# cbs228/sameold

Hardware: AMD Instinct MI355X
Metric: Msamples/s demodulated (batched 22.05 kHz channels) + % HBM roofline, 1/8 GPU (higher is better)
Workload: dtype f32

## Files before the change

### sameold_amd/csrc/same_batch.cpp

```cpp
#include <hip/hip_runtime.h>

#include <algorithm>
#include <chrono>
#include <cstdarg>
#include <cstdio>
#include <cstdlib>
#include <condition_variable>
#include <cstring>
#include <deque>
#include <functional>
#include <mutex>
#include <new>
#include <string>
#include <thread>
#include <utility>
#include <vector>

#include "../../include/same_rx.h"
#include "same_config.h"
#include "same_device.h"
#include "same_hipmem.h"
#include "same_launch.h"
#include "same_resets.h"
#include "same_transport.h"
// ... 191 lines not shown
        uint64_t end_counter = 0;
        bool chunked = false;
        same::ChunkGeom geom{};
        uint64_t end_blocks = 0;
        same::DevBuf<uint64_t> d_handover;
        same::PinnedBuf<uint64_t> h_handover;
        bool per_channel = false;
        same::DevBuf<uint32_t> d_geom;
        same::PinnedBuf<uint32_t> h_geom;
        same::CoherentBuf<uint32_t> h_reset;
        same::CoherentBuf<uint32_t> h_counts;
        same::PinnedBuf<uint64_t> h_wake_up;
        bool dev_transport = false;
        same::CoherentBuf<same::DevMessage> h_near;
        uint32_t near_cap() const { return (uint32_t)h_near.size(); }
        same::DevBuf<same::DevMessage> d_msgs;
        uint32_t msg_cap() const { return (uint32_t)d_msgs.size(); }
        same::PinnedBuf<void> h_msgs;
        bool captured = false;
        same::DevBuf<same::cap::Span> d_spans;
        uint32_t span_cap() const { return (uint32_t)d_spans.size(); }
        same::DevBuf<float> d_pool;
        same::DevBuf<same::cap::Cursors> d_cap_cur;
        same::MappedBuf<same::cap::Cursors> h_cap_cur;
        same::PinnedBuf<void> h_spans, h_pool;
    } slot[2];
    struct TimePar {
        bool enabled = false;
        uint32_t max_chunks = 0, min_own = 0, warmup = 0;
        uint32_t cap_columns = 0;
        uint32_t carved_columns = 0;
        int carved_family = -1;
        same::Params Pv{};
        same::State Sv{};
        same::DevBuf<void> blob;
        same::DevBuf<void> blob_fresh;
        size_t fresh_bytes = 0;
        same::DevBuf<same::StateArrayDesc> d_desc_in, d_desc_out;
        uint32_t n_desc = 0;
        same::DevBuf<uint32_t> d_final_col;
        same::DevBuf<float> d_energy;
        same::DevBuf<float> d_hist;
        same::Event ev_plan_prev; bool plan_recorded = false;
        int knob_plan_stream = 0;
        int sort_mode = -1;
        uint32_t last_chunks = 1;
        bool last_per_channel = false;
        same::Family family = same::Family::kPipe;
        int knob_prologue = 0;
        std::vector<int64_t> sym_off;
        std::vector<TickSynth> synth;
    } tp;
    uint64_t launch_seq = 0;
    hipStream_t copy_stream = nullptr;
    struct Windowed {
        bool on = false;
        uint32_t window = 0;
        uint32_t fill = 0;
        same::DevBuf<void> d_buf;
        same::Event ev_buf;
        hipStream_t buf_stream = nullptr; bool buf_used = false;
        same::Event ev_read[2];
        uint64_t n_reads = 0;
        hipStream_t read_stream = nullptr;
    } inv;
    hipStream_t plan_stream = nullptr;
    float last_ms = 0.0f;
    bool overflowed = false;
    std::string record_path;
    bool kernel_fault = false;
    same::Request want;
    same::Mode mode;
    same::Choice plain;
    same::Params Pfm{};
    same::Family last_family = same::Family::kGeneric;
    bool sym_launched = false;
    bool debug = false;
    int host_threads = 0;
    same::DevBuf<void> d_stage, d_stage2;
    same::DevBuf<void> d_upload;
    same::DevBuf<void> d_zero;
    same::Event ev_order;
// ... 94 lines not shown
{
    out.clear();
#define DESC_ROWS(field, type, rows)                                                                     \
    out.push_back(same::StateArrayDesc{reinterpret_cast<char *>(src.field), reinterpret_cast<char *>(dst.field), \
                                       (uint32_t)(rows), (uint32_t)(sizeof(type) / 4)});
    SAME_STATE_ARRAYS(DESC_ROWS, P)
#undef DESC_ROWS
    static_assert(same::kBurstCap % 4 == 0, "framer rows are copied in words");
    out.push_back(same::StateArrayDesc{reinterpret_cast<char *>(src.fr_msg), reinterpret_cast<char *>(dst.fr_msg), 1u,
                                       (uint32_t)(same::kBurstCap / 4)});
}

void read_knobs(same_batch *rx)
{
    auto num = [](const char *name, int unset) { const char *e = std::getenv(name); return e ? std::atoi(e) : unset; };
    auto tri = [](const char *name) { const char *e = std::getenv(name); return e ? (std::atoi(e) ? 1 : -1) : 0; };
    rx->P.knob_pipe = tri("SAME_PIPE");
    rx->P.knob_pipe_lanes = num("SAME_PIPE_LANES", 0);
    rx->P.knob_pipe_split = tri("SAME_PIPE_SPLIT");
#ifdef SAME_PROFILE
    rx->P.knob_mirror = tri("SAME_MIRROR");
    rx->P.knob_pipe_share = tri("SAME_PIPE_SHARE");
    rx->P.knob_prio = num("SAME_PIPE_PRIO", 0);
#endif
    rx->P.knob_fast_dense = tri("SAME_FAST_DENSE");
    rx->P.knob_sym = tri("SAME_SYM");
    rx->want.sym_max_channels = (uint32_t)std::max(0, num("SAME_SYM_MAX", 1 << 30));
    rx->debug = std::getenv("SAME_DEBUG") != nullptr;
    { const char *e = std::getenv("SAME_RECORD_HARVEST"); rx->record_path = e ? e : ""; }
    rx->host_threads = std::max(0, num("SAME_HOST_THREADS", 0));
    rx->tp.sort_mode = num("SAME_TP_SORT", -1);
    rx->tp.knob_plan_stream = tri("SAME_TP_PLAN_STREAM");
    rx->tp.knob_prologue = tri("SAME_TP_PROLOGUE");
    rx->want.knob_relaxed = tri("SAME_RELAXED");
    { const char *e = std::getenv("SAME_RELAXED_KERNEL"); rx->P.knob_relaxed_kernel = !e ? 0 : (std::strcmp(e, "solo") == 0 ? 1 : (std::strcmp(e, "duo") == 0 ? 2 : 0)); }
    { const char *e = std::getenv("SAME_TP_KERNEL"); rx->want.knob_tp_kernel = !e ? 0 : (std::strcmp(e, "wave") == 0 ? 2 : (std::strcmp(e, "pipe") == 0 ? 1 : 0)); }
}

int ensure_output(same_batch *rx, same_batch::Slot &sl, size_t n_samples, same::Output &O, size_t n_columns = 0)
{
    const size_t n_ch = n_columns ? n_columns : rx->P.n_channels;
    const double symbols = (double)n_samples * 520.83 / (double)rx->P.input_rate;
    const size_t per_chan_events = (size_t)(symbols / 8.0) + 16;
    const size_t per_chan_bursts = (size_t)(symbols / 160.0) + 4;
    size_t ecap = std::min<size_t>(per_chan_events * n_ch, 0x7fffffffu / sizeof(same::DevEvent));
    size_t bcap = std::min<size_t>(per_chan_bursts * n_ch, 0x7fffffffu / same::kBurstCap);
    HIP_TRY(sl.d_events.ensure(ecap));
    HIP_TRY(sl.d_bursts.ensure(bcap * same::kBurstCap));
    if (rx->dev_transport && !n_columns) {
        HIP_TRY(sl.d_msgs.ensure(std::min<size_t>(bcap + 2 * n_ch, 0x7fffffffu / sizeof(same::DevMessage))));
        if (!sl.h_near) HIP_TRY(sl.h_near.ensure(std::max<uint32_t>(4096u, (uint32_t)(n_ch / 4u))));
        if (rx->audio.per_launch)
            HIP_TRY(sl.d_spans.ensure(std::min<size_t>(n_ch + (size_t)sl.near_cap() + sl.msg_cap(), 0x7fffffffu / sizeof(same::cap::Span))));
    }
    HIP_TRY(sl.d_sorted.ensure(sl.d_events.size()));
    HIP_TRY(sl.d_sort.ensure(2 * n_ch + 1 + same::event_sort_extra_words((uint32_t)n_ch)));
    HIP_TRY(sl.h_sort.ensure(n_ch + 1));
    sl.sort_bins = (uint32_t)n_ch;
    O.events = sl.d_events; O.event_cap = sl.event_cap();
    O.bursts = sl.d_bursts; O.burst_cap = sl.burst_cap();
    O.n_events = sl.d_counters; O.n_bursts = sl.d_counters + 1; O.overflow = sl.d_counters + 2;
    return SAME_OK;
}

template <typename SampleT>
hipError_t launch_family(same::Family f, const same::Params &P, const same::State &S, const same::Output &O, const float4 *taps, const SampleT *x,
// ... 618 lines not shown
        const uint64_t min_own = tp.min_own ? tp.min_own : 4ull * WB * fb;
        if (SB == 0 || SB * fb < min_own) return false;
        geom.counter0 = rx->counter;
        geom.n_chunks = K; geom.block_len = fb; geom.stride_blocks = (uint32_t)SB; geom.warmup_blocks = WB;
        pc.n_chunks = K; pc.in_channels = C; pc.stride_blocks = (uint32_t)SB; pc.nominal_blocks = (uint32_t)SB + WB;
        pc.handover = nullptr;
        return true;
    };
    const same::TpRule rule = same::tp_rule(rx->P, rx->mode, rx->want, tp.max_chunks, column_cap, channel_major);
    for (uint32_t K = rule.k_max; K >= 2u; --K) {
        same::Choice c;
        if (same::tp_candidate(rx->P, rule, K, c) && fill(K, c.block_len)) { tp.family = c.family; return K; }
    }
    return 1;
}

int ensure_handover(same_batch::Slot &sl, uint32_t columns)
{
    HIP_TRY(sl.d_handover.ensure(columns));
    HIP_TRY(sl.h_handover.ensure(columns));
    return SAME_OK;
}

int ensure_wide_state(same_batch *rx, uint32_t columns)
{
    same_batch::TimePar &tp = rx->tp;
    if (tp.carved_columns == columns && tp.carved_family == (int)tp.family) return SAME_OK;
    int rc = harvest(rx);
    if (rc) return rc;
    HIP_TRY(hipDeviceSynchronize());
    tp.Pv = same::wide_params(rx->P, columns, same::is_fastmath(tp.family), same::tp_more_than_one_round(columns));
    if (columns > tp.cap_columns) {
        tp.cap_columns = 0;
        HIP_TRY(tp.blob.reset());
        HIP_TRY(tp.blob_fresh.reset());
        const size_t bytes = carve_state(tp.Pv, nullptr, tp.Sv);
        HIP_TRY(tp.blob.ensure(bytes));
        HIP_TRY(hipMemset(tp.blob, 0, bytes));
        HIP_TRY(tp.blob_fresh.ensure(bytes));
        tp.cap_columns = columns;
    }
    const size_t blob_bytes = carve_state(tp.Pv, (char *)tp.blob.get(), tp.Sv);
    {
        same::State Sf{};
        carve_state(tp.Pv, (char *)tp.blob_fresh.get(), Sf);
        HIP_TRY(hipMemset(tp.blob_fresh, 0, blob_bytes));
        HIP_TRY(same::launch_init_state(tp.Pv, Sf, 0, nullptr, 0));
        HIP_TRY(hipDeviceSynchronize());
        tp.fresh_bytes = (size_t)(reinterpret_cast<char *>(tp.Sv.fr_msg) - static_cast<char *>(tp.blob.get()));
    }
    std::vector<same::StateArrayDesc> in, out;
    list_state_arrays(rx->P, rx->S, tp.Sv, in);
    list_state_arrays(rx->P, tp.Sv, rx->S, out);
    tp.n_desc = (uint32_t)in.size();
    HIP_TRY(tp.d_desc_in.ensure(in.size()));
    HIP_TRY(tp.d_desc_out.ensure(out.size()));
    HIP_TRY(tp.d_final_col.ensure(rx->P.n_channels));
    HIP_TRY(hipMemcpy(tp.d_desc_in, in.data(), in.size() * sizeof(same::StateArrayDesc), hipMemcpyHostToDevice));
    HIP_TRY(hipMemcpy(tp.d_desc_out, out.data(), out.size() * sizeof(same::StateArrayDesc), hipMemcpyHostToDevice));
    tp.carved_columns = columns;
    tp.carved_family = (int)tp.family;
    return SAME_OK;
}

struct Ragged {
    const uint32_t *counts = nullptr;
    uint32_t m = 0;
    uint32_t row_off = 0;
};

struct RaggedLaunch {
    uint32_t row0 = 0;
    size_t n_lock = 0;
};


int begin_launch(same_batch *rx, same_batch::Slot &sl, const same_batch::Slot &prev, hipStream_t stream)
{
    int rc = harvest_slot(rx, sl);
    if (rc) return rc;
    if (prev.in_flight && rx->last_stream != stream) HIP_TRY(hipStreamWaitEvent(stream, prev.ev_done, 0));
    return launch_pending_resets(rx, sl, stream);
}

int begin_timing(same_batch *rx, same_batch::Slot &sl, hipStream_t stream)
{
    sl.timed = rx->timing;
    if (sl.timed) HIP_TRY(hipEventRecord(sl.ev_start, stream));
    return SAME_OK;
}

int tp_reserve(same_batch *rx, same_batch::Slot &sl, uint32_t columns, size_t n, const same::PipeChunks &pc, uint32_t block_len, same::Output &O)
{
    int rc = ensure_wide_state(rx, columns);
    if (rc) return rc;
    rc = ensure_output(rx, sl, std::min<size_t>(n, 3 * (size_t)pc.nominal_blocks * block_len + 65536), O, columns);
    if (rc) return rc;
    return ensure_handover(sl, columns);
}

int tp_start(same_batch *rx, same_batch::Slot &sl, uint32_t columns, const char *layout, hipStream_t stream, bool *sort_bins_empty)
{
    same_batch::TimePar &tp = rx->tp;
    const uint32_t C = rx->P.n_channels;
    *sort_bins_empty = false;
    if (tp.knob_prologue >= 0) {
        HIP_TRY(same::launch_tp_prologue(tp.blob, tp.blob_fresh, tp.fresh_bytes, sl.d_handover, sl.d_sort, columns, sl.d_counters, stream));
        *sort_bins_empty = sl.sort_bins == columns;
    } else {
        HIP_TRY(same::launch_counters(sl.d_counters, sl.h_counters.dev(), 0, stream));
        HIP_TRY(same::launch_init_state(tp.Pv, tp.Sv, 0, stream, C));
        HIP_TRY(same::launch_fill_u64(sl.d_handover, columns, same::kNoHandover, stream));
    }
    if (rx->debug) std::fprintf(stderr, "[same] time-parallel launch: %u columns (%s), start-up: %s\n", columns, layout,
                                tp.knob_prologue >= 0 ? "prologue kernel" : "separate launches");
    HIP_TRY(same::launch_copy_state_columns(tp.d_desc_in, tp.n_desc, C, columns, nullptr, C, stream));
    return SAME_OK;
}

int tp_hand_back(same_batch *rx, same_batch::Slot &sl, const same::ChunkGeom &geom, const uint32_t *own_start, hipStream_t stream)
{
    same_batch::TimePar &tp = rx->tp;
    const uint32_t C = rx->P.n_channels;
    if (own_start) HIP_TRY(same::launch_chunk_final_column_pc(sl.d_handover, own_start, C, geom.n_chunks, rx->counter, tp.d_final_col, stream));
    else HIP_TRY(same::launch_chunk_final_column(sl.d_handover, C, geom, tp.d_final_col, stream));
    HIP_TRY(same::launch_copy_state_columns(tp.d_desc_out, tp.n_desc, geom.n_chunks * C, C, tp.d_final_col, C, stream));
    return SAME_OK;
}

template <typename SampleT>
int demod_tail(same_batch *rx, const same::Output &O, const SampleT *rows, size_t n, uint64_t counter0, hipStream_t stream)
{
    const hipError_t e = same::launch_demod(rx->P, rx->S, O, rx->d_taps, rows, (uint32_t)n, counter0, stream);
    if (e != hipSuccess) return fail(SAME_EHIP, "demod kernel launch failed: %s", hipGetErrorString(e));
    return SAME_OK;
}
int demod_tail_corner(same_batch *rx, const same::Output &O, const float *corner, size_t pitch, size_t r, uint64_t counter0, hipStream_t stream)
{
    const uint32_t C = rx->P.n_channels;
    HIP_TRY(rx->d_stage.ensure(r * C * sizeof(float)));
    HIP_TRY(rx->d_stage2.ensure(r * C * sizeof(float)));
    float *staged = static_cast<float *>(rx->d_stage.get()), *rows = static_cast<float *>(rx->d_stage2.get());
    HIP_TRY(hipMemcpy2DAsync(staged, r * sizeof(float), corner, pitch * sizeof(float), r * sizeof(float), C, hipMemcpyDeviceToDevice, stream));
    const hipError_t e = same::launch_transpose(staged, rows, C, (uint32_t)r, stream);
    if (e != hipSuccess) return fail(SAME_EHIP, "demod kernel launch failed: %s", hipGetErrorString(e));
    return demod_tail(rx, O, rows, r, counter0, stream);
}

template <typename SampleT>
int end_launch(same_batch *rx, same_batch::Slot &sl, same_batch::Slot &prev, hipStream_t stream, const SampleT *rows, size_t n,
               bool sort_bins_empty, const RaggedLaunch *rl = nullptr)
{
    if (sl.timed) HIP_TRY(hipEventRecord(sl.ev_stop, stream));
    HIP_TRY(same::launch_event_sort(sl.d_events, sl.d_counters, sl.event_cap(), sl.sort_bins, sl.d_sort, sl.d_sort + sl.sort_bins,
                                    sl.d_sorted, stream, sort_bins_empty));
    sl.dev_transport = rx->dev_transport && !sl.chunked;
    rx->last_dev_transport = sl.dev_transport;
    if (sl.dev_transport) {
        same::TransportLaunch T{};
// ... 44 lines not shown
        same_batch::Slot &sl = rx->slot[rx->launch_seq & 1];
        same_batch::Slot &prev = rx->slot[(rx->launch_seq & 1) ^ 1];
        int rc = begin_launch(rx, sl, prev, stream);
        if (rc) return rc;
        size_t n_lock = n;
        if (rg) {
            const size_t row0 = (size_t)rg->row_off + done;
            n_lock = rg->m > row0 ? std::min<size_t>(rg->m - row0, n) : 0;
            const uint32_t C = rx->P.n_channels;
            HIP_TRY(sl.h_counts.ensure(C));
            std::memcpy(sl.h_counts, rg->counts, (size_t)C * sizeof(uint32_t));
            rx->ragged_by.resize(C);
            for (uint32_t c = 0; c < C; ++c) {
                const size_t have = rg->counts[c] > row0 ? std::min<size_t>(rg->counts[c] - row0, n) : 0;
                rx->ragged_by[c] = (uint32_t)(n - have);
            }
        }
        same::ChunkGeom geom{};
        same::PipeChunks pc{};
        const uint32_t n_chunks = rg ? 1u : plan_chunks(rx, n, geom, pc);
        rx->tp.last_chunks = n_chunks;
        sl.have_k = false;
        bool sort_bins_empty = false;
        same::Output O{};
        if (n_chunks > 1u) {
            const uint32_t C = rx->P.n_channels, columns = n_chunks * C;
            const size_t fbk = geom.block_len;
            rc = tp_reserve(rx, sl, columns, n, pc, geom.block_len, O);
            if (rc) return rc;
            pc.handover = sl.d_handover;
            same_batch::TimePar &tp = rx->tp;
            rc = begin_timing(rx, sl, stream);
            if (rc) return rc;
            rc = tp_start(rx, sl, columns, "time-major", stream, &sort_bins_empty);
            if (rc) return rc;
            const SampleT *xp = d_x + done * C;
            const uint32_t total_blocks = (uint32_t)(n / fbk);
            const hipError_t e = launch_family(tp.family, tp.Pv, tp.Sv, O, rx->d_taps, xp, total_blocks, rx->counter, stream, pc);
            rx->last_family = tp.family;
            if (e != hipSuccess) return fail(SAME_EHIP, "time-parallel demod kernel launch failed: %s", hipGetErrorString(e));
            rc = tp_hand_back(rx, sl, geom, nullptr, stream);
            if (rc) return rc;
            const size_t n_whole = (size_t)total_blocks * fbk;
            if (n_whole < n && (rc = demod_tail(rx, O, xp + n_whole * C, n - n_whole, rx->counter + n_whole, stream)) != SAME_OK) return rc;
            sl.chunked = true; sl.per_channel = false;
            sl.geom = geom;
            sl.end_blocks = rx->counter + n_whole;
            rx->tp.last_per_channel = false;
        } else {
        sl.chunked = false; sl.per_channel = false;
        rc = ensure_output(rx, sl, n, O);
        if (rc) return rc;
        HIP_TRY(same::launch_counters(sl.d_counters, sl.h_counters.dev(), 0, stream));
        rc = begin_timing(rx, sl, stream);
        if (rc) return rc;
        const SampleT *xp = d_x + done * rx->P.n_channels;
        hipError_t e = hipSuccess;
        const same::Choice &plain = rx->plain;
        const size_t fb = plain.block_len;
        const size_t n_fast = fb ? (n_lock / fb) * fb : 0;
        if (n_fast) {
            e = launch_family(plain.family, same::is_fastmath(plain.family) ? rx->Pfm : rx->P, rx->S, O, rx->d_taps, xp, (uint32_t)(n_fast / fb), rx->counter, stream);
            if (e != hipSuccess) return fail(SAME_EHIP, "%s launch failed: %s", same::family_name(plain.family, rx->P.block_len), hipGetErrorString(e));
            rx->sym_launched |= plain.family == same::Family::kSym;
        }
        rx->last_family = plain.family == same::Family::kSym && !rx->sym_launched ? same::Family::kPipeFastmath : plain.family;
        if (n_fast < n_lock &&
            (rc = demod_tail(rx, O, xp + n_fast * rx->P.n_channels, n_lock - n_fast, rx->counter + n_fast, stream)) != SAME_OK) return rc;
        if (n_lock < n) {
            e = same::launch_demod_ragged(rx->P, rx->S, O, rx->d_taps, xp + n_lock * rx->P.n_channels, (uint32_t)(n - n_lock), sl.h_counts.dev(),
                                          (uint32_t)(rg->row_off + done + n_lock), rx->counter + n_lock, stream);
// ... 129 lines not shown
    int rc = begin_launch(rx, sl, prev, stream);
    if (rc) return rc;
    same::Output O{};
    rc = tp_reserve(rx, sl, columns, n, pc, fb, O);
    if (rc) return rc;
    HIP_TRY(sl.d_geom.ensure((size_t)5 * columns + 3 * (columns / same::kWave)));
    HIP_TRY(sl.h_geom.ensure((size_t)2 * columns));
    same::TpPlan plan{};
    plan.channels = C; plan.n_chunks = n_chunks; plan.block_len = fb;
    {
        const double sps = (double)rx->P.input_rate / 520.83;
        const uint32_t warm = tp.warmup ? tp.warmup : (uint32_t)(40.0 * sps + 0.5);
        plan.warmup_samples = std::min(geom.warmup_blocks, (warm + fb - 1u) / fb) * fb;
    }
    plan.whole_samples = (uint32_t)n; plan.in_samples = n_call;
    plan.scout_blocks = (uint32_t)(n / same::tp_scout_block());
    HIP_TRY(tp.d_energy.ensure((size_t)C * plan.scout_blocks));
    uint32_t *d_own = sl.d_geom, *d_row0 = sl.d_geom + columns, *d_nom = sl.d_geom + 2 * (size_t)columns,
             *d_perm = sl.d_geom + 3 * (size_t)columns, *d_wg = sl.d_geom + 4 * (size_t)columns,
             *d_wg2 = d_wg + columns / same::kWave, *d_perm2 = d_wg2 + 2 * (columns / same::kWave);
    const bool pair_groups = tp.sort_mode == 2 && tp.family == same::Family::kSym;
    const int sort_mode = pair_groups ? 0 : (tp.sort_mode >= 0 ? (tp.sort_mode ? 1 : 0) : (same::tp_more_than_one_round(columns) ? 1 : 0));
    rc = begin_timing(rx, sl, stream);
    if (rc) return rc;
    const bool lpt = sort_mode != 0 || pair_groups;
    const bool side = stream == rx->own_stream && tp.knob_plan_stream >= 0;
    hipStream_t ps = side ? rx->plan_stream : stream;
    if (tp.plan_recorded) HIP_TRY(hipStreamWaitEvent(ps, tp.ev_plan_prev, 0));
    HIP_TRY(same::launch_tp_plan(d_x, plan, tp.d_energy, d_own, d_row0, d_nom, d_perm, d_wg, sort_mode != 0, ps,
                                 lpt ? d_perm2 : nullptr, lpt ? d_wg2 : nullptr, pair_groups));
    HIP_TRY(tp.ev_plan_prev.ensure());
    HIP_TRY(hipEventRecord(tp.ev_plan_prev, ps));
    tp.plan_recorded = true;
    if (side) {
        HIP_TRY(hipEventRecord(sl.ev_planned, ps));
        HIP_TRY(hipStreamWaitEvent(stream, sl.ev_planned, 0));
    }
    if (lpt) { d_perm = d_perm2; d_wg = d_wg2; }
    bool sort_bins_empty = false;
    rc = tp_start(rx, sl, columns, "channel-major", stream, &sort_bins_empty);
    if (rc) return rc;
    pc.handover = sl.d_handover;
    pc.col_row0 = d_row0; pc.col_nominal = d_nom; pc.wg_blocks = d_wg; pc.col_perm = (sort_mode != 0 || pair_groups) ? d_perm : nullptr;
    pc.in_samples = n_call; pc.whole_samples = (uint32_t)n;
    pc.hist_scratch = nullptr;
    if (pc.col_perm && tp.family == same::Family::kSym) {
        HIP_TRY(tp.d_hist.ensure((size_t)columns * same::kSquelchHist));
        pc.hist_scratch = tp.d_hist;
    }
    sl.have_k = sl.timed;
    if (sl.timed) HIP_TRY(hipEventRecord(sl.ev_k0, stream));
    const hipError_t e = launch_family(tp.family, tp.Pv, tp.Sv, O, rx->d_taps, d_x, (uint32_t)(n / fb), rx->counter, stream, pc);
    rx->last_family = tp.family;
    if (e != hipSuccess) return fail(SAME_EHIP, "time-parallel demod kernel launch failed: %s", hipGetErrorString(e));
    if (sl.timed) HIP_TRY(hipEventRecord(sl.ev_k1, stream));
    rc = tp_hand_back(rx, sl, geom, d_own, stream);
    if (rc) return rc;
    if (n < n_call && (rc = demod_tail_corner(rx, O, d_x + n, n_call, n_call - n, rx->counter + n, stream)) != SAME_OK) return rc;
    sl.chunked = true; sl.per_channel = true;
    sl.geom = geom;
    sl.end_blocks = rx->counter + n;
    tp.last_chunks = n_chunks; tp.last_per_channel = true;
    rc = end_launch<float>(rx, sl, prev, stream, nullptr, n_call, sort_bins_empty);
    return rc ? rc : 1;
}
int process_channel_major_native(same_batch *, const int16_t *, size_t, hipStream_t) { return 0; }

template <typename SampleT, typename Launch>
int transpose_in_slabs(same_batch *rx, const SampleT *d_x, size_t pitch, size_t n_rows, hipStream_t stream, Launch &&launch)
{
    const uint32_t C = rx->P.n_channels;
    for (same_batch::Slot &sl : rx->slot)
        if (sl.in_flight && rx->last_stream != stream) HIP_TRY(hipStreamWaitEvent(stream, sl.ev_done, 0));
    const size_t slab = std::min<size_t>(n_rows, (size_t)65520);
    HIP_TRY(rx->d_stage2.ensure(slab * C * sizeof(SampleT)));
    for (size_t t0 = 0; t0 < n_rows; t0 += slab) {
        const size_t n = std::min(slab, n_rows - t0);
        HIP_TRY(rx->d_stage.ensure(n * C * sizeof(SampleT)));
        SampleT *staged = static_cast<SampleT *>(rx->d_stage.get()), *rows = static_cast<SampleT *>(rx->d_stage2.get());
        HIP_TRY(hipMemcpy2DAsync(staged, n * sizeof(SampleT), d_x + t0, pitch * sizeof(SampleT), n * sizeof(SampleT), C,
                                 hipMemcpyDeviceToDevice, stream));
        const hipError_t e = same::launch_transpose(staged, rows, C, (uint32_t)n, stream);
        if (e != hipSuccess) return fail(SAME_EHIP, "transpose launch failed: %s", hipGetErrorString(e));
        const int rc = launch(rows, n, t0);
        if (rc) return rc;
// ... 852 lines not shown
```

### sameold_amd/csrc/same_kernels.hip

```cpp
#include <hip/hip_runtime.h>

#include <algorithm>

#include "same_dev_common.h"
#include "same_device.h"
#include "same_launch.h"

namespace same {

template <int B, typename SampleT>
__global__ __launch_bounds__(kWave) void demod_kernel(Params P, State S, Output O,
                                                      const float4 *__restrict__ taps,
                                                      const SampleT *__restrict__ x,
                                                      uint32_t n_samples, uint64_t counter0)
{
    extern __shared__ float lds[];
    const uint32_t lane = threadIdx.x;
    const uint32_t C = P.n_channels;
    const uint32_t c_raw = blockIdx.x * kWave + lane;
    if (c_raw >= C) return;
    const uint32_t c = c_raw;
    const uint32_t DL = P.dc_len;
    float *ff = lds;
    float *fb = lds + DL * kWave;
// ... 419 lines not shown
}

hipError_t launch_reset_columns(const Params &P, const State &S, const uint32_t *cols, uint32_t n, hipStream_t stream)
{
    if (!n) return hipSuccess;
    hipLaunchKernelGGL(reset_columns_kernel, dim3((n + 63u) / 64u), dim3(64), 0, stream, P, S, cols, n);
    return hipGetLastError();
}

__global__ void copy_state_columns_kernel(const StateArrayDesc *desc, uint32_t Csrc, uint32_t Cdst,
                                          const uint32_t *src_col, uint32_t n_cols, uint32_t src_base)
{
    const uint32_t col = blockIdx.x * blockDim.x + threadIdx.x;
    if (col >= n_cols) return;
    const StateArrayDesc d = desc[blockIdx.y];
    const uint32_t sc = src_col ? src_col[col] : col + src_base;
    const uint32_t w = d.elem_words;
    const uint32_t *src = reinterpret_cast<const uint32_t *>(d.src);
    uint32_t *dst = reinterpret_cast<uint32_t *>(d.dst);
    const uint32_t n = d.rows * w;
    for (uint32_t k = blockIdx.z; k < n; k += gridDim.z) {
        const uint32_t r = k / w, i = k - r * w;
        dst[((size_t)r * Cdst + col) * w + i] = src[((size_t)r * Csrc + sc) * w + i];
    }
}
hipError_t launch_copy_state_columns(const StateArrayDesc *desc, uint32_t n_desc, uint32_t src_channels,
                                     uint32_t dst_channels, const uint32_t *src_col, uint32_t n_cols, hipStream_t stream,
                                     uint32_t src_base)
{
    hipLaunchKernelGGL(copy_state_columns_kernel, dim3((n_cols + 255) / 256, n_desc, 16), dim3(256), 0, stream, desc,
                       src_channels, dst_channels, src_col, n_cols, src_base);
    return hipGetLastError();
}
__global__ void chunk_final_column_kernel(const uint64_t *handover, uint32_t C, ChunkGeom g, uint32_t *final_col)
{
    const uint32_t c = blockIdx.x * blockDim.x + threadIdx.x;
    if (c >= C) return;
    uint32_t cur = 0;
    for (;;) {
        const uint64_t h = handover[(size_t)cur * C + c];
        if (h == kNoHandover) break;
        const uint32_t nxt = g.owner_of(h);
        if (nxt <= cur) break;
        cur = nxt;
    }
    final_col[c] = cur * C + c;
}
hipError_t launch_chunk_final_column(const uint64_t *handover, uint32_t in_channels, ChunkGeom g, uint32_t *final_col,
                                     hipStream_t stream)
{
    hipLaunchKernelGGL(chunk_final_column_kernel, dim3((in_channels + 255) / 256), dim3(256), 0, stream, handover, in_channels, g, final_col);
    return hipGetLastError();
}
__global__ void chunk_final_column_pc_kernel(const uint64_t *handover, const uint32_t *own_start, uint32_t C, uint32_t K,
                                             uint64_t counter0, uint32_t *final_col)
{
    const uint32_t c = blockIdx.x * blockDim.x + threadIdx.x;
    if (c >= C) return;
    uint32_t cur = 0;
    for (;;) {
        const uint64_t h = handover[(size_t)cur * C + c];
        if (h == kNoHandover) break;
        uint32_t nxt = cur;
        for (uint32_t k = cur + 1u; k < K; ++k)
            if (counter0 + own_start[(size_t)k * C + c] <= h) nxt = k;
        if (nxt <= cur) break;
        cur = nxt;
    }
    final_col[c] = cur * C + c;
}
hipError_t launch_chunk_final_column_pc(const uint64_t *handover, const uint32_t *own_start, uint32_t in_channels, uint32_t n_chunks,
                                        uint64_t counter0, uint32_t *final_col, hipStream_t stream)
{
    hipLaunchKernelGGL(chunk_final_column_pc_kernel, dim3((in_channels + 255) / 256), dim3(256), 0, stream, handover, own_start,
                       in_channels, n_chunks, counter0, final_col);
    return hipGetLastError();
}
#ifndef SAME_SCOUT_BLOCK
#define SAME_SCOUT_BLOCK 256
#endif
constexpr uint32_t kScoutBlock = SAME_SCOUT_BLOCK;
uint32_t tp_scout_block() { return kScoutBlock; }
__global__ void tp_scout_kernel(const float *__restrict__ x, TpPlan g, float *__restrict__ energy)
{
    const size_t t = (size_t)blockIdx.x * blockDim.x + threadIdx.x;
    const size_t i = t >> 2;
    const uint32_t q = (uint32_t)t & 3u;
    const bool live = i < (size_t)g.channels * g.scout_blocks;
    float e = 0.0f;
    if (live) {
        const uint32_t c = (uint32_t)(i / g.scout_blocks), j = (uint32_t)(i % g.scout_blocks);
        const float4 v = reinterpret_cast<const float4 *>(x + (size_t)c * g.in_samples + (size_t)j * kScoutBlock)[q];
        e = (fabsf(v.x) + fabsf(v.y)) + (fabsf(v.z) + fabsf(v.w));
    }
    e += __shfl_xor(e, 1);
    e += __shfl_xor(e, 2);
    if (live && q == 0u) energy[i] = e;
}
__global__ __launch_bounds__(kWave) void tp_boundaries_kernel(const float *__restrict__ energy, TpPlan g, uint32_t *__restrict__ own_start,
                                                               uint32_t *__restrict__ row0, uint32_t *__restrict__ nominal)
{
    extern __shared__ float tp_lds[];
    const uint32_t c = blockIdx.x, lane = threadIdx.x;
    const int NB = (int)g.scout_blocks, K = (int)g.n_chunks;
    float *e = tp_lds;
    int *lastq = reinterpret_cast<int *>(tp_lds + NB);
    int *cut = lastq + NB;
    constexpr int kQuietBefore = 2048 / (int)kScoutBlock, kQuietAfter = 1;
// ... 223 lines not shown
```

### sameold_amd/csrc/same_launch.h

```cpp
#pragma once

#include <hip/hip_runtime.h>

#include "same_capture_dev.h"
#include "same_device.h"
#include "same_select.h"

namespace same {

hipError_t launch_demod(const Params &P, const State &S, const Output &O, const float4 *taps,
                        const float *x, uint32_t n_samples, uint64_t counter0, hipStream_t stream);
hipError_t launch_demod(const Params &P, const State &S, const Output &O, const float4 *taps,
                        const int16_t *x, uint32_t n_samples, uint64_t counter0, hipStream_t stream);
hipError_t launch_demod_ragged(const Params &P, const State &S, const Output &O, const float4 *taps, const float *x,
                               uint32_t n_rows, const uint32_t *counts, uint32_t row_sub, uint64_t counter0, hipStream_t stream);
hipError_t launch_demod_ragged(const Params &P, const State &S, const Output &O, const float4 *taps, const int16_t *x,
                               uint32_t n_rows, const uint32_t *counts, uint32_t row_sub, uint64_t counter0, hipStream_t stream);
hipError_t launch_demod_pipe(const Params &P, const State &S, const Output &O, const float4 *taps,
                             const float *x, uint32_t n_blocks, uint64_t counter0, hipStream_t stream,
                             const PipeChunks &chunks = PipeChunks{}, bool relaxed = false);
hipError_t launch_demod_pipe(const Params &P, const State &S, const Output &O, const float4 *taps,
                             const int16_t *x, uint32_t n_blocks, uint64_t counter0, hipStream_t stream,
                             const PipeChunks &chunks = PipeChunks{}, bool relaxed = false);
hipError_t launch_demod_sym(const Params &P, const State &S, const Output &O, const float4 *taps,
                            const float *x, uint32_t n_blocks, uint64_t counter0, hipStream_t stream,
                            const PipeChunks &chunks = PipeChunks{});
hipError_t launch_demod_sym(const Params &P, const State &S, const Output &O, const float4 *taps,
                            const int16_t *x, uint32_t n_blocks, uint64_t counter0, hipStream_t stream,
                            const PipeChunks &chunks = PipeChunks{});
hipError_t launch_demod_relaxed(const Params &P, const State &S, const Output &O, const float4 *taps,
                                const float *x, uint32_t n_blocks, uint64_t counter0, hipStream_t stream,
                                const PipeChunks &chunks = PipeChunks{});
hipError_t launch_demod_relaxed(const Params &P, const State &S, const Output &O, const float4 *taps,
                                const int16_t *x, uint32_t n_blocks, uint64_t counter0, hipStream_t stream,
                                const PipeChunks &chunks = PipeChunks{});
hipError_t launch_demod_fast(const Params &P, const State &S, const Output &O, const float4 *taps,
                             const float *x, uint32_t n_blocks, uint64_t counter0, hipStream_t stream);
hipError_t launch_demod_fast(const Params &P, const State &S, const Output &O, const float4 *taps,
                             const int16_t *x, uint32_t n_blocks, uint64_t counter0, hipStream_t stream);
hipError_t launch_counters(uint32_t *dev, uint32_t *host_mapped, int publish, hipStream_t stream);
uint32_t event_sort_extra_words(uint32_t n_bins);
hipError_t launch_event_sort(const DevEvent *ev, const uint32_t *counters, uint32_t cap, uint32_t n_bins, uint32_t *cnt, uint32_t *first,
                             DevEvent *sorted, hipStream_t stream, bool cnt_is_zero = false);
hipError_t launch_init_state(const Params &P, const State &S, int is_reset, hipStream_t stream, uint32_t first_col = 0);
hipError_t launch_reset_columns(const Params &P, const State &S, const uint32_t *cols, uint32_t n, hipStream_t stream);
hipError_t launch_copy_state_columns(const StateArrayDesc *desc, uint32_t n_desc, uint32_t src_channels,
                                     uint32_t dst_channels, const uint32_t *src_col, uint32_t n_cols, hipStream_t stream,
                                     uint32_t src_base = 0);
hipError_t launch_chunk_final_column(const uint64_t *handover, uint32_t in_channels, ChunkGeom g, uint32_t *final_col,
                                     hipStream_t stream);
hipError_t launch_chunk_final_column_pc(const uint64_t *handover, const uint32_t *own_start, uint32_t in_channels, uint32_t n_chunks,
                                        uint64_t counter0, uint32_t *final_col, hipStream_t stream);
hipError_t launch_fill_u64(uint64_t *p, size_t n, uint64_t v, hipStream_t stream);
hipError_t launch_cast_i16_f32(const int16_t *in, float *out, size_t n, hipStream_t stream);
hipError_t launch_tp_prologue(void *blob, const void *fresh, size_t bytes, uint64_t *handover, uint32_t *sort_cnt, uint32_t n_cols,
                              uint32_t *counters, hipStream_t stream);
uint32_t tp_scout_block();
struct TpPlan {
    uint32_t channels, n_chunks, block_len, warmup_samples, whole_samples;
    uint64_t in_samples;
    uint32_t scout_blocks;
};
hipError_t launch_tp_plan(const float *x, const TpPlan &g, float *energy, uint32_t *own_start, uint32_t *row0,
                          uint32_t *nominal, uint32_t *perm, uint32_t *wg_blocks, bool sorted, hipStream_t stream,
                          uint32_t *perm_out = nullptr, uint32_t *wg_blocks_out = nullptr, bool pairs = false);
hipError_t launch_transpose(const float *in, float *out, uint32_t n_channels, uint32_t n_samples,
                            hipStream_t stream);
hipError_t launch_transpose(const int16_t *in, int16_t *out, uint32_t n_channels, uint32_t n_samples,
                            hipStream_t stream);

constexpr uint32_t kMessageLogOverflow = 8u;
struct TransportLaunch {
    uint32_t n_channels, input_rate;
    const uint32_t *first;
    DevEvent *sorted;
    const uint32_t *counters;
    const uint8_t *bursts; uint32_t burst_cap;
    void *hot, *cold;
    uint64_t *wake_sample;
    DevMessage *near; uint32_t near_cap;
    DevMessage *log; uint32_t log_cap;
    uint32_t *log_cursor, *overflow;
    cap::Launch cap;
};
size_t transport_hot_bytes();
// ... 31 lines not shown
```

Before: 467,400.

## Double-buffer wide state per slot, overlap prologue on plan stream, fuse hand-back

Result: slower. 459,000 (-1.8%).

```diff
diff --git a/sameold_amd/csrc/same_batch.cpp b/sameold_amd/csrc/same_batch.cpp
--- a/sameold_amd/csrc/same_batch.cpp
+++ b/sameold_amd/csrc/same_batch.cpp
@@ -247,13 +247,15 @@
         uint32_t carved_columns = 0;
         int carved_family = -1;
         same::Params Pv{};
-        same::State Sv{};
-        same::DevBuf<void> blob;
+        struct Wide {
+            same::State Sv{};
+            same::DevBuf<void> blob;
+            same::DevBuf<same::StateArrayDesc> d_desc_in, d_desc_out;
+            same::DevBuf<uint32_t> d_final_col;
+        } wide[2];
         same::DevBuf<void> blob_fresh;
         size_t fresh_bytes = 0;
-        same::DevBuf<same::StateArrayDesc> d_desc_in, d_desc_out;
         uint32_t n_desc = 0;
-        same::DevBuf<uint32_t> d_final_col;
         same::DevBuf<float> d_energy;
         same::DevBuf<float> d_hist;
         same::Event ev_plan_prev; bool plan_recorded = false;
@@ -263,6 +265,8 @@
         bool last_per_channel = false;
         same::Family family = same::Family::kPipe;
         int knob_prologue = 0;
+        int knob_prologue_side = 0;
+        int knob_handback = 0;
         std::vector<int64_t> sym_off;
         std::vector<TickSynth> synth;
     } tp;
@@ -423,6 +427,8 @@
     rx->tp.sort_mode = num("SAME_TP_SORT", -1);
     rx->tp.knob_plan_stream = tri("SAME_TP_PLAN_STREAM");
     rx->tp.knob_prologue = tri("SAME_TP_PROLOGUE");
+    rx->tp.knob_prologue_side = tri("SAME_TP_PROLOGUE_SIDE");
+    rx->tp.knob_handback = tri("SAME_TP_HANDBACK");
     rx->want.knob_relaxed = tri("SAME_RELAXED");
     { const char *e = std::getenv("SAME_RELAXED_KERNEL"); rx->P.knob_relaxed_kernel = !e ? 0 : (std::strcmp(e, "solo") == 0 ? 1 : (std::strcmp(e, "duo") == 0 ? 2 : 0)); }
     { const char *e = std::getenv("SAME_TP_KERNEL"); rx->want.knob_tp_kernel = !e ? 0 : (std::strcmp(e, "wave") == 0 ? 2 : (std::strcmp(e, "pipe") == 0 ? 1 : 0)); }
@@ -1107,32 +1113,37 @@
     tp.Pv = same::wide_params(rx->P, columns, same::is_fastmath(tp.family), same::tp_more_than_one_round(columns));
     if (columns > tp.cap_columns) {
         tp.cap_columns = 0;
-        HIP_TRY(tp.blob.reset());
+        for (same_batch::TimePar::Wide &w : tp.wide) HIP_TRY(w.blob.reset());
         HIP_TRY(tp.blob_fresh.reset());
-        const size_t bytes = carve_state(tp.Pv, nullptr, tp.Sv);
-        HIP_TRY(tp.blob.ensure(bytes));
-        HIP_TRY(hipMemset(tp.blob, 0, bytes));
+        const size_t bytes = carve_state(tp.Pv, nullptr, tp.wide[0].Sv);
+        for (same_batch::TimePar::Wide &w : tp.wide) {
+            HIP_TRY(w.blob.ensure(bytes));
+            HIP_TRY(hipMemset(w.blob, 0, bytes));
+        }
         HIP_TRY(tp.blob_fresh.ensure(bytes));
         tp.cap_columns = columns;
     }
-    const size_t blob_bytes = carve_state(tp.Pv, (char *)tp.blob.get(), tp.Sv);
+    size_t blob_bytes = 0;
+    for (same_batch::TimePar::Wide &w : tp.wide) blob_bytes = carve_state(tp.Pv, (char *)w.blob.get(), w.Sv);
     {
         same::State Sf{};
         carve_state(tp.Pv, (char *)tp.blob_fresh.get(), Sf);
         HIP_TRY(hipMemset(tp.blob_fresh, 0, blob_bytes));
         HIP_TRY(same::launch_init_state(tp.Pv, Sf, 0, nullptr, 0));
         HIP_TRY(hipDeviceSynchronize());
-        tp.fresh_bytes = (size_t)(reinterpret_cast<char *>(tp.Sv.fr_msg) - static_cast<char *>(tp.blob.get()));
-    }
-    std::vector<same::StateArrayDesc> in, out;
-    list_state_arrays(rx->P, rx->S, tp.Sv, in);
-    list_state_arrays(rx->P, tp.Sv, rx->S, out);
-    tp.n_desc = (uint32_t)in.size();
-    HIP_TRY(tp.d_desc_in.ensure(in.size()));
-    HIP_TRY(tp.d_desc_out.ensure(out.size()));
-    HIP_TRY(tp.d_final_col.ensure(rx->P.n_channels));
-    HIP_TRY(hipMemcpy(tp.d_desc_in, in.data(), in.size() * sizeof(same::StateArrayDesc), hipMemcpyHostToDevice));
-    HIP_TRY(hipMemcpy(tp.d_desc_out, out.data(), out.size() * sizeof(same::StateArrayDesc), hipMemcpyHostToDevice));
+        tp.fresh_bytes = (size_t)(reinterpret_cast<char *>(Sf.fr_msg) - static_cast<char *>(tp.blob_fresh.get()));
+    }
+    for (same_batch::TimePar::Wide &w : tp.wide) {
+        std::vector<same::StateArrayDesc> in, out;
+        list_state_arrays(rx->P, rx->S, w.Sv, in);
+        list_state_arrays(rx->P, w.Sv, rx->S, out);
+        tp.n_desc = (uint32_t)in.size();
+        HIP_TRY(w.d_desc_in.ensure(in.size()));
+        HIP_TRY(w.d_desc_out.ensure(out.size()));
+        HIP_TRY(w.d_final_col.ensure(rx->P.n_channels));
+        HIP_TRY(hipMemcpy(w.d_desc_in, in.data(), in.size() * sizeof(same::StateArrayDesc), hipMemcpyHostToDevice));
+        HIP_TRY(hipMemcpy(w.d_desc_out, out.data(), out.size() * sizeof(same::StateArrayDesc), hipMemcpyHostToDevice));
+    }
     tp.carved_columns = columns;
     tp.carved_family = (int)tp.family;
     return SAME_OK;
@@ -1174,32 +1185,47 @@
     return ensure_handover(sl, columns);
 }
 
-int tp_start(same_batch *rx, same_batch::Slot &sl, uint32_t columns, const char *layout, hipStream_t stream, bool *sort_bins_empty)
+same_batch::TimePar::Wide &tp_wide(same_batch *rx, const same_batch::Slot &sl) { return rx->tp.wide[&sl - rx->slot]; }
+
+int tp_fresh_columns(same_batch *rx, same_batch::Slot &sl, uint32_t columns, hipStream_t stream, bool *sort_bins_empty)
 {
     same_batch::TimePar &tp = rx->tp;
-    const uint32_t C = rx->P.n_channels;
+    same_batch::TimePar::Wide &w = tp_wide(rx, sl);
     *sort_bins_empty = false;
     if (tp.knob_prologue >= 0) {
-        HIP_TRY(same::launch_tp_prologue(tp.blob, tp.blob_fresh, tp.fresh_bytes, sl.d_handover, sl.d_sort, columns, sl.d_counters, stream));
+        HIP_TRY(same::launch_tp_prologue(w.blob, tp.blob_fresh, tp.fresh_bytes, sl.d_handover, sl.d_sort, columns, sl.d_counters, stream));
         *sort_bins_empty = sl.sort_bins == columns;
     } else {
         HIP_TRY(same::launch_counters(sl.d_counters, sl.h_counters.dev(), 0, stream));
-        HIP_TRY(same::launch_init_state(tp.Pv, tp.Sv, 0, stream, C));
+        HIP_TRY(same::launch_init_state(tp.Pv, w.Sv, 0, stream, rx->P.n_channels));
         HIP_TRY(same::launch_fill_u64(sl.d_handover, columns, same::kNoHandover, stream));
     }
-    if (rx->debug) std::fprintf(stderr, "[same] time-parallel launch: %u columns (%s), start-up: %s\n", columns, layout,
-                                tp.knob_prologue >= 0 ? "prologue kernel" : "separate launches");
-    HIP_TRY(same::launch_copy_state_columns(tp.d_desc_in, tp.n_desc, C, columns, nullptr, C, stream));
-    return SAME_OK;
-}
-
-int tp_hand_back(same_batch *rx, same_batch::Slot &sl, const same::ChunkGeom &geom, const uint32_t *own_start, hipStream_t stream)
+    return SAME_OK;
+}
+
+int tp_start(same_batch *rx, same_batch::Slot &sl, uint32_t columns, const char *layout, hipStream_t stream, bool beside)
 {
     same_batch::TimePar &tp = rx->tp;
     const uint32_t C = rx->P.n_channels;
-    if (own_start) HIP_TRY(same::launch_chunk_final_column_pc(sl.d_handover, own_start, C, geom.n_chunks, rx->counter, tp.d_final_col, stream));
-    else HIP_TRY(same::launch_chunk_final_column(sl.d_handover, C, geom, tp.d_final_col, stream));
-    HIP_TRY(same::launch_copy_state_columns(tp.d_desc_out, tp.n_desc, geom.n_chunks * C, C, tp.d_final_col, C, stream));
+    if (rx->debug) std::fprintf(stderr, "[same] time-parallel launch: %u columns (%s), start-up: %s, copy-in; hand-back: %s\n", columns, layout,
+                                tp.knob_prologue < 0 ? "separate launches" : (beside ? "prologue kernel on the plan stream" : "prologue kernel"),
+                                tp.knob_handback >= 0 ? "one kernel" : "two launches");
+    HIP_TRY(same::launch_copy_state_columns(tp_wide(rx, sl).d_desc_in, tp.n_desc, C, columns, nullptr, C, stream));
+    return SAME_OK;
+}
+
+int tp_hand_back(same_batch *rx, same_batch::Slot &sl, const same::ChunkGeom &geom, const uint32_t *own_start, hipStream_t stream)
+{
+    same_batch::TimePar &tp = rx->tp;
+    same_batch::TimePar::Wide &w = tp_wide(rx, sl);
+    const uint32_t C = rx->P.n_channels;
+    if (tp.knob_handback >= 0) {
+        HIP_TRY(same::launch_tp_hand_back(w.d_desc_out, tp.n_desc, sl.d_handover, own_start, C, geom, stream));
+        return SAME_OK;
+    }
+    if (own_start) HIP_TRY(same::launch_chunk_final_column_pc(sl.d_handover, own_start, C, geom.n_chunks, rx->counter, w.d_final_col, stream));
+    else HIP_TRY(same::launch_chunk_final_column(sl.d_handover, C, geom, w.d_final_col, stream));
+    HIP_TRY(same::launch_copy_state_columns(w.d_desc_out, tp.n_desc, geom.n_chunks * C, C, w.d_final_col, C, stream));
     return SAME_OK;
 }
 
@@ -1310,11 +1336,13 @@
             same_batch::TimePar &tp = rx->tp;
             rc = begin_timing(rx, sl, stream);
             if (rc) return rc;
-            rc = tp_start(rx, sl, columns, "time-major", stream, &sort_bins_empty);
+            rc = tp_fresh_columns(rx, sl, columns, stream, &sort_bins_empty);
+            if (rc) return rc;
+            rc = tp_start(rx, sl, columns, "time-major", stream, false);
             if (rc) return rc;
             const SampleT *xp = d_x + done * C;
             const uint32_t total_blocks = (uint32_t)(n / fbk);
-            const hipError_t e = launch_family(tp.family, tp.Pv, tp.Sv, O, rx->d_taps, xp, total_blocks, rx->counter, stream, pc);
+            const hipError_t e = launch_family(tp.family, tp.Pv, tp_wide(rx, sl).Sv, O, rx->d_taps, xp, total_blocks, rx->counter, stream, pc);
             rx->last_family = tp.family;
             if (e != hipSuccess) return fail(SAME_EHIP, "time-parallel demod kernel launch failed: %s", hipGetErrorString(e));
             rc = tp_hand_back(rx, sl, geom, nullptr, stream);
@@ -1510,13 +1538,16 @@
     HIP_TRY(tp.ev_plan_prev.ensure());
     HIP_TRY(hipEventRecord(tp.ev_plan_prev, ps));
     tp.plan_recorded = true;
+    const bool beside = side && tp.knob_prologue >= 0 && tp.knob_prologue_side >= 0;
+    bool sort_bins_empty = false;
+    if (beside && (rc = tp_fresh_columns(rx, sl, columns, ps, &sort_bins_empty)) != SAME_OK) return rc;
     if (side) {
         HIP_TRY(hipEventRecord(sl.ev_planned, ps));
         HIP_TRY(hipStreamWaitEvent(stream, sl.ev_planned, 0));
     }
     if (lpt) { d_perm = d_perm2; d_wg = d_wg2; }
-    bool sort_bins_empty = false;
-    rc = tp_start(rx, sl, columns, "channel-major", stream, &sort_bins_empty);
+    if (!beside && (rc = tp_fresh_columns(rx, sl, columns, stream, &sort_bins_empty)) != SAME_OK) return rc;
+    rc = tp_start(rx, sl, columns, "channel-major", stream, beside);
     if (rc) return rc;
     pc.handover = sl.d_handover;
     pc.col_row0 = d_row0; pc.col_nominal = d_nom; pc.wg_blocks = d_wg; pc.col_perm = (sort_mode != 0 || pair_groups) ? d_perm : nullptr;
@@ -1528,7 +1559,7 @@
     }
     sl.have_k = sl.timed;
     if (sl.timed) HIP_TRY(hipEventRecord(sl.ev_k0, stream));
-    const hipError_t e = launch_family(tp.family, tp.Pv, tp.Sv, O, rx->d_taps, d_x, (uint32_t)(n / fb), rx->counter, stream, pc);
+    const hipError_t e = launch_family(tp.family, tp.Pv, tp_wide(rx, sl).Sv, O, rx->d_taps, d_x, (uint32_t)(n / fb), rx->counter, stream, pc);
     rx->last_family = tp.family;
     if (e != hipSuccess) return fail(SAME_EHIP, "time-parallel demod kernel launch failed: %s", hipGetErrorString(e));
     if (sl.timed) HIP_TRY(hipEventRecord(sl.ev_k1, stream));
diff --git a/sameold_amd/csrc/same_kernels.hip b/sameold_amd/csrc/same_kernels.hip
--- a/sameold_amd/csrc/same_kernels.hip
+++ b/sameold_amd/csrc/same_kernels.hip
@@ -475,10 +475,8 @@
                        src_channels, dst_channels, src_col, n_cols, src_base);
     return hipGetLastError();
 }
-__global__ void chunk_final_column_kernel(const uint64_t *handover, uint32_t C, ChunkGeom g, uint32_t *final_col)
-{
-    const uint32_t c = blockIdx.x * blockDim.x + threadIdx.x;
-    if (c >= C) return;
+__device__ __forceinline__ uint32_t final_chunk(const uint64_t *handover, uint32_t C, uint32_t c, const ChunkGeom &g)
+{
     uint32_t cur = 0;
     for (;;) {
         const uint64_t h = handover[(size_t)cur * C + c];
@@ -487,19 +485,11 @@
         if (nxt <= cur) break;
         cur = nxt;
     }
-    final_col[c] = cur * C + c;
-}
-hipError_t launch_chunk_final_column(const uint64_t *handover, uint32_t in_channels, ChunkGeom g, uint32_t *final_col,
-                                     hipStream_t stream)
-{
-    hipLaunchKernelGGL(chunk_final_column_kernel, dim3((in_channels + 255) / 256), dim3(256), 0, stream, handover, in_channels, g, final_col);
-    return hipGetLastError();
-}
-__global__ void chunk_final_column_pc_kernel(const uint64_t *handover, const uint32_t *own_start, uint32_t C, uint32_t K,
-                                             uint64_t counter0, uint32_t *final_col)
-{
-    const uint32_t c = blockIdx.x * blockDim.x + threadIdx.x;
-    if (c >= C) return;
+    return cur;
+}
+__device__ __forceinline__ uint32_t final_chunk_pc(const uint64_t *handover, const uint32_t *own_start, uint32_t C, uint32_t K,
+                                                   uint32_t c, uint64_t counter0)
+{
     uint32_t cur = 0;
     for (;;) {
         const uint64_t h = handover[(size_t)cur * C + c];
@@ -510,13 +500,60 @@
         if (nxt <= cur) break;
         cur = nxt;
     }
-    final_col[c] = cur * C + c;
+    return cur;
+}
+__global__ void chunk_final_column_kernel(const uint64_t *handover, uint32_t C, ChunkGeom g, uint32_t *final_col)
+{
+    const uint32_t c = blockIdx.x * blockDim.x + threadIdx.x;
+    if (c >= C) return;
+    final_col[c] = final_chunk(handover, C, c, g) * C + c;
+}
+hipError_t launch_chunk_final_column(const uint64_t *handover, uint32_t in_channels, ChunkGeom g, uint32_t *final_col,
+                                     hipStream_t stream)
+{
+    hipLaunchKernelGGL(chunk_final_column_kernel, dim3((in_channels + 255) / 256), dim3(256), 0, stream, handover, in_channels, g, final_col);
+    return hipGetLastError();
+}
+__global__ void chunk_final_column_pc_kernel(const uint64_t *handover, const uint32_t *own_start, uint32_t C, uint32_t K,
+                                             uint64_t counter0, uint32_t *final_col)
+{
+    const uint32_t c = blockIdx.x * blockDim.x + threadIdx.x;
+    if (c >= C) return;
+    final_col[c] = final_chunk_pc(handover, own_start, C, K, c, counter0) * C + c;
 }
 hipError_t launch_chunk_final_column_pc(const uint64_t *handover, const uint32_t *own_start, uint32_t in_channels, uint32_t n_chunks,
                                         uint64_t counter0, uint32_t *final_col, hipStream_t stream)
 {
     hipLaunchKernelGGL(chunk_final_column_pc_kernel, dim3((in_channels + 255) / 256), dim3(256), 0, stream, handover, own_start,
                        in_channels, n_chunks, counter0, final_col);
+    return hipGetLastError();
+}
+constexpr uint32_t kHandBackSlices = 32;
+__global__ __launch_bounds__(256) void tp_hand_back_kernel(const StateArrayDesc *__restrict__ desc, uint32_t n_desc,
+                                                           const uint64_t *__restrict__ handover, const uint32_t *__restrict__ own_start,
+                                                           uint32_t C, ChunkGeom g)
+{
+    const uint32_t c = blockIdx.x * blockDim.x + threadIdx.x;
+    if (c >= C) return;
+    const uint32_t K = g.n_chunks;
+    const uint32_t sc = (own_start ? final_chunk_pc(handover, own_start, C, K, c, g.counter0) : final_chunk(handover, C, c, g)) * C + c;
+    const size_t Csrc = (size_t)K * C;
+    for (uint32_t di = 0; di < n_desc; ++di) {
+        const StateArrayDesc d = desc[di];
+        const uint32_t w = d.elem_words, n = d.rows * w;
+        const uint32_t *src = reinterpret_cast<const uint32_t *>(d.src);
+        uint32_t *dst = reinterpret_cast<uint32_t *>(d.dst);
+        for (uint32_t k = (blockIdx.y + gridDim.y - di % gridDim.y) % gridDim.y; k < n; k += gridDim.y) {
+            const uint32_t r = k / w, i = k - r * w;
+            dst[((size_t)r * C + c) * w + i] = src[((size_t)r * Csrc + sc) * w + i];
+        }
+    }
+}
+hipError_t launch_tp_hand_back(const StateArrayDesc *desc, uint32_t n_desc, const uint64_t *handover, const uint32_t *own_start,
+                               uint32_t in_channels, ChunkGeom g, hipStream_t stream)
+{
+    hipLaunchKernelGGL(tp_hand_back_kernel, dim3((in_channels + 255) / 256, kHandBackSlices), dim3(256), 0, stream, desc, n_desc,
+                       handover, own_start, in_channels, g);
     return hipGetLastError();
 }
 #ifndef SAME_SCOUT_BLOCK
diff --git a/sameold_amd/csrc/same_launch.h b/sameold_amd/csrc/same_launch.h
--- a/sameold_amd/csrc/same_launch.h
+++ b/sameold_amd/csrc/same_launch.h
@@ -51,6 +51,8 @@
                                      hipStream_t stream);
 hipError_t launch_chunk_final_column_pc(const uint64_t *handover, const uint32_t *own_start, uint32_t in_channels, uint32_t n_chunks,
                                         uint64_t counter0, uint32_t *final_col, hipStream_t stream);
+hipError_t launch_tp_hand_back(const StateArrayDesc *desc, uint32_t n_desc, const uint64_t *handover, const uint32_t *own_start,
+                               uint32_t in_channels, ChunkGeom g, hipStream_t stream);
 hipError_t launch_fill_u64(uint64_t *p, size_t n, uint64_t v, hipStream_t stream);
 hipError_t launch_cast_i16_f32(const int16_t *in, float *out, size_t n, hipStream_t stream);
 hipError_t launch_tp_prologue(void *blob, const void *fresh, size_t bytes, uint64_t *handover, uint32_t *sort_cnt, uint32_t n_cols,
```
